# PKU-MARL/HARL

Hardware: AMD Instinct MI355X
Metric: transitions/sec through HAPPO update (MPE spread, 3 agents) (higher is better)
Workload: dtype f32; 1 GPU; MPE simple_spread_v2 3-agent HAPPO update: compute_returns + train(), T=200, n_rollout_threads=4096/GPU (4096 global, weak scaling), obs18/share54/Box5, MLP[128, 128], ppo_epoch=5, critic_epoch=5; episode_length=200, n_rollout_threads_per_gpu=4096, n_rollout_threads_global=4096, n_agents=3, parallelism=dp1, collective=none, world_size=1, ranks_seen=1

## Files before the change

harl_amd/csrc/heads_common.h:

```cpp
#pragma once
#include "common.h"

using namespace harl;

namespace {
constexpr float LOG_SQRT_2PI = 0.918938533204672741780329736406f;
constexpr float HALF_LOG_2PI_PLUS_HALF = 1.418938533204672741780329736406f;

struct ActorArgs {
  const float *xL;
  const uint32_t *relu_mask;
  const float *rstd;
  long M;
  const float *Whp, *bhp, *log_std;
  float std_x_coef, std_y_coef;
  int act_dim;
  const int64_t *idx;
  const float *actions, *avail, *old_logp, *adv;
  const double *adv_moments;
  const float *factor_in, *active;
  float clip_lo, clip_hi, entropy_coef;
  int agg_mean;
  float *dzL, *dhead, *part_scalars;
  float *dw_part;
// ... 75 lines not shown
        dx += dzh[4 * dq + 0] * w[0] + dzh[4 * dq + 1] * w[1] + dzh[4 * dq + 2] * w[2] + dzh[4 * dq + 3] * w[3];
      }
      const float da = rstd * (dx - s1 - xv[c] * s2);
      o[c] = (int)b0 < 0 ? da : 0.f;
      b0 <<= 1;
    }
    op[q * WAVE] = o;
    xv = xn;
  }
}

template <int H>
__device__ __forceinline__ void head_load_regs(const float *__restrict__ xL, long slab, int lane, f32x4 (&xs)[H / 8]) {
  const f32x4 *xp = reinterpret_cast<const f32x4 *>(xL + slab * (long)(H * SLAB)) + lane;
#pragma unroll
  for (int q = 0; q < H / 8; ++q) xs[q] = xp[q * WAVE];
}

template <int H, int DAP, int DA = DAP>
__device__ __forceinline__ void head_fwd_regs(const f32x4 (&xs)[H / 8], const float *whl_h, const float *cst,
                                              float (&z)[DAP]) {
#pragma unroll
  for (int d = 0; d < DAP; ++d) z[d] = 0.f;
#pragma unroll
  for (int q = 0; q < H / 8; ++q) {
#pragma unroll
    for (int c = 0; c < 4; ++c) {
#pragma unroll
      for (int dq = 0; dq < (DA + 3) / 4; ++dq) {
        const f32x4 w = *reinterpret_cast<const f32x4 *>(whl_h + (4 * q + c) * DAP + 4 * dq);
#pragma unroll
        for (int e = 0; e < 4; ++e)
          if (4 * dq + e < DA) z[4 * dq + e] += xs[q][c] * w[e];
      }
    }
    __builtin_amdgcn_sched_barrier(0);
  }
#pragma unroll
  for (int d = 0; d < DA; ++d) z[d] = wave_sum32(z[d]) + cst[d];
}

constexpr int HEAD_T_PAD = 16;
__host__ __device__ constexpr int head_t_rows(int da) { return 2 * ((da + 1) / 2); }
__host__ __device__ constexpr int head_t_block(int H, int da) { return head_t_rows(da) * (H / 2) + HEAD_T_PAD; }

template <int H, int DAP, int DA>
__device__ __forceinline__ void head_fwd_regs_t(const f32x4 (&xs)[H / 8], const float *whlT_h, const float *cst,
                                                float (&z)[DAP]) {
#pragma unroll
  for (int d = 0; d < DAP; ++d) z[d] = 0.f;
  f32x4 w[2][DA];
#pragma unroll
  for (int d = 0; d < DA; ++d) w[0][d] = *reinterpret_cast<const f32x4 *>(whlT_h + d * (H / 2));
#pragma unroll
  for (int q = 0; q < H / 8; ++q) {
    if (q + 1 < H / 8) {
#pragma unroll
      for (int d = 0; d < DA; ++d) w[(q + 1) & 1][d] = *reinterpret_cast<const f32x4 *>(whlT_h + d * (H / 2) + 4 * (q + 1));
    }
#pragma unroll
    for (int c = 0; c < 4; ++c)
#pragma unroll
      for (int d = 0; d < DA; ++d) z[d] += xs[q][c] * w[q & 1][d][c];
    __builtin_amdgcn_sched_barrier(0);
  }
#pragma unroll
  for (int d = 0; d < DA; ++d) z[d] = wave_sum32(z[d]) + cst[d];
}

template <int H, int DAP, int DA>
__device__ __forceinline__ void stage_head_t(float *whlT, float *cst, const float *__restrict__ Whp,
                                             const float *__restrict__ bhp, int n_threads) {
  constexpr int DAE = head_t_rows(DA), BLK = head_t_block(H, DA);
  for (int e = threadIdx.x; e < 2 * DAE * (H / 2); e += n_threads) {
    const int R = e % (H / 2), d = (e / (H / 2)) % DAE, hh = e / ((H / 2) * DAE);
    whlT[hh * BLK + d * (H / 2) + R] = d < DA ? Whp[d * H + feat_base(R) + 4 * hh] : 0.f;
  }
  for (int e = threadIdx.x; e < DAP; e += n_threads) {
    cst[e] = e < DA ? bhp[e] : 0.f;
    float rs = 0.f;
    if (e < DA)
      for (int f = 0; f < H; ++f) rs += Whp[e * H + f];
    cst[4 * DAP + e] = rs;
  }
}

template <int H, int DAP, int DA = DAP, bool PACKED = false, bool WT = false>
__device__ __forceinline__ void head_bwd_regs_bits(const f32x4 (&xs)[H / 8], uint32_t b0, const uint32_t b1, float rstd,
                                                   long slab, int lane, const float *whl ,
                                                   const float (&dzh)[DAP], float s1, float s2,
                                                   float *__restrict__ dz_out, const uint32_t bm1 = 0u,
                                                   const uint32_t bm2 = 0u) {
  s1 *= (1.0f / H);
  s2 *= (1.0f / H);
  const int i = lane & 31, h = lane >> 5;
  const float *wa = WT ? whl + ((i >> 2) & 1) * head_t_block(H, DA) + (i & 3) + 4 * (i >> 3) + h * (H / 2)
                       : whl + (((i >> 2) & 1) * (H / 2) + (i & 3) + 4 * (i >> 3)) * DAP + h;
  f32x16 acc[H / 32];
#pragma unroll
  for (int t = 0; t < H / 32; ++t)
#pragma unroll
    for (int r = 0; r < 16; ++r) acc[t][r] = 0.f;
#pragma unroll
  for (int st = 0; st < (DA + 1) / 2; ++st) {
    const unsigned hm = 0u - (unsigned)h;
    const float bsel = __uint_as_float((__float_as_uint(dzh[2 * st + 1]) & hm) | (__float_as_uint(dzh[2 * st]) & ~hm));
#pragma unroll
    for (int t = 0; t < H / 32; ++t)
      acc[t] = __builtin_amdgcn_mfma_f32_32x32x2f32(wa[WT ? 16 * t + 2 * st * (H / 2) : 16 * t * DAP + 2 * st], bsel, acc[t], 0, 0, 0);
  }
  f32x4 *op = reinterpret_cast<f32x4 *>(dz_out + slab * (long)(H * SLAB)) + lane;
  const float c1 = -s1 * rstd, c2 = -s2 * rstd;
  const f32x2 c1v = {c1, c1}, c2v = {c2, c2}, rv = {rstd, rstd};
#pragma unroll
  for (int q = 0; q < H / 8; ++q) {
    if (q == 8) b0 = H == 256 ? bm1 : b1;
    if (H == 256 && q == 16) b0 = bm2;
    if (H == 256 && q == 24) b0 = b1;
    f32x4 o;
    if constexpr (PACKED) {
#pragma unroll
      for (int P = 0; P < 2; ++P) {
        const int e = 4 * q + 2 * P;
        const f32x2 d = {acc[e >> 4][e & 15], acc[(e + 1) >> 4][(e + 1) & 15]}, x = {xs[q][2 * P], xs[q][2 * P + 1]};
        const f32x2 da = fma2(x, c2v, fma2(d, rv, c1v));
        o[2 * P] = mask_pop(da[0], b0);
        o[2 * P + 1] = mask_pop(da[1], b0);
      }
    } else {
#pragma unroll
      for (int c = 0; c < 4; ++c) {
        const float dx = acc[(4 * q + c) >> 4][(4 * q + c) & 15];
        const float da = rstd * (dx - s1 - xs[q][c] * s2);
        o[c] = (int)b0 < 0 ? da : 0.f;
        b0 <<= 1;
      }
    }
    op[q * WAVE] = o;
  }
}

template <int H, int DAP>
__device__ __forceinline__ void head_bwd_regs(const f32x4 (&xs)[H / 8], const uint32_t *__restrict__ mask_in,
                                              float rstd, long slab, int lane, const float *whl ,
                                              const float (&dzh)[DAP], float s1, float s2,
                                              float *__restrict__ dz_out) {
  constexpr int NW = (H / 2 + 31) / 32;
  const uint32_t b0 = mask_in[(slab * NW + 0) * WAVE + lane];
  const uint32_t b1 = NW > 1 ? mask_in[(slab * NW + (NW - 1)) * WAVE + lane] : 0u;
  const uint32_t bm1 = NW == 4 ? mask_in[(slab * NW + 1) * WAVE + lane] : 0u, bm2 = NW == 4 ? mask_in[(slab * NW + 2) * WAVE + lane] : 0u;
  head_bwd_regs_bits<H, DAP>(xs, b0, b1, rstd, slab, lane, whl, dzh, s1, s2, dz_out, bm1, bm2);
}

template <int H>
struct HeadDw {
  static constexpr int HX = 64 + 4;
  static constexpr int TD = 33;
  static constexpr int WAVE_FLOATS = SLAB * HX + SLAB * TD;
  static constexpr int OUT_FLOATS = 32 * H + 32;
};

template <int H, int DAP>
__device__ __forceinline__ void head_dw_step(const f32x4 (&xs)[H / 8], const float (&dzh)[DAP], float *tx, float *td,
                                             int lane, f32x16 (&acc)[H / 32]) {
  constexpr int HX = HeadDw<H>::HX, TD = HeadDw<H>::TD;
  const int i = lane & 31, h = lane >> 5;
  if (h == 0) {
#pragma unroll
    for (int d = 0; d < DAP; ++d) td[i * TD + d] = dzh[d];
  }
#pragma unroll
  for (int half = 0; half < H / 64; ++half) {
#pragma unroll
    for (int q = 0; q < 8; ++q)
      *reinterpret_cast<f32x4 *>(tx + i * HX + 32 * (q >> 2) + 8 * (q & 3) + 4 * h) = xs[8 * half + q];
    asm volatile("s_waitcnt lgkmcnt(0)" ::: "memory");
    __builtin_amdgcn_wave_barrier();
#pragma unroll
    for (int t = 0; t < SLAB / 2; ++t) {
      const float a = td[(2 * t + h) * TD + i];
#pragma unroll
      for (int n = 0; n < 2; ++n) {
        const float b = tx[(2 * t + h) * HX + 32 * n + i];
        acc[2 * half + n] = __builtin_amdgcn_mfma_f32_32x32x2f32(a, b, acc[2 * half + n], 0, 0, 0);
      }
    }
    asm volatile("s_waitcnt lgkmcnt(0)" ::: "memory");
    __builtin_amdgcn_wave_barrier();
  }
}

template <int H, int DAP, int HROWS>
__device__ __forceinline__ void head_dw_step_lds(const f32x4 (&xs)[H / 8], const float (&dzh)[DAP], float *tx, float *td,
                                                 int lane, float *hw) {
  constexpr int HX = HeadDw<H>::HX, TD = HeadDw<H>::TD;
  static_assert(HROWS <= 8, "rows 0..7 of a 16 x 16 tile live in the four registers of lane groups 0 and 1");
  const int i = lane & 31, h = lane >> 5;
  const int m16 = lane & 15, kg = lane >> 4;
  if (h == 0) {
#pragma unroll
    for (int d = 0; d < DAP; ++d) td[i * TD + d] = dzh[d];
  }
#pragma unroll
  for (int half = 0; half < H / 64; ++half) {
#pragma unroll
    for (int q = 0; q < 8; ++q)
      *reinterpret_cast<f32x4 *>(tx + i * HX + 32 * (q >> 2) + 8 * (q & 3) + 4 * h) = xs[8 * half + q];
    asm volatile("s_waitcnt lgkmcnt(0)" ::: "memory");
    __builtin_amdgcn_wave_barrier();
    f32x4 acc[4];
#pragma unroll
    for (int n = 0; n < 4; ++n) acc[n] = f32x4{0.f, 0.f, 0.f, 0.f};
#pragma unroll
    for (int t = 0; t < SLAB / 4; ++t) {
      const float a = td[(4 * t + kg) * TD + m16];
#pragma unroll
      for (int n = 0; n < 4; ++n) {
        const float b = tx[(4 * t + kg) * HX + 16 * n + m16];
        acc[n] = __builtin_amdgcn_mfma_f32_16x16x4f32(a, b, acc[n], 0, 0, 0);
      }
    }
#pragma unroll
    for (int n = 0; n < 4; ++n)
#pragma unroll
      for (int r = 0; r < 4; ++r) {
        if (r < HROWS && kg == 0) hw[r * H + 64 * half + 16 * n + m16] += acc[n][r];
        if (4 + r < HROWS && kg == 1) hw[(4 + r) * H + 64 * half + 16 * n + m16] += acc[n][r];
      }
    asm volatile("s_waitcnt lgkmcnt(0)" ::: "memory");
    __builtin_amdgcn_wave_barrier();
  }
}

template <int H, int DAP, int HROWS, int NWAVES>
__device__ __forceinline__ void head_dw_finish_lds(const float *hacc, float (&dbacc)[DAP], float *dbl,
                                                   float *__restrict__ out) {
  const int lane = threadIdx.x & 63, wave = wave_id();
  float dbs[DAP];
#pragma unroll
  for (int d = 0; d < DAP; ++d) dbs[d] = wave_reduce_sum(dbacc[d]);
  __syncthreads();
  if (lane == 0) {
#pragma unroll
    for (int d = 0; d < DAP; ++d) dbl[wave * PS_STRIDE + d] = dbs[d];
  }
  __syncthreads();
  for (int e = threadIdx.x; e < HeadDw<H>::OUT_FLOATS; e += 64 * NWAVES) {
    float t = 0.f;
    if (e < 32 * H) {
      const int row = e / H;
      if (row < HROWS) {
#pragma unroll
        for (int w = 0; w < NWAVES; ++w) t += hacc[(w * HROWS + row) * H + (e - row * H)];
      }
    } else {
      const int d = e - 32 * H;
      if (d < DAP) {
#pragma unroll
        for (int w = 0; w < NWAVES; ++w) t += dbl[w * PS_STRIDE + d];
      }
    }
    out[e] = t;
  }
}

template <int H, int DAP>
__device__ __forceinline__ void head_dw_finish(f32x16 (&acc)[H / 32], float (&dbacc)[DAP], float *buf ,
                                               float *__restrict__ out) {
  const int lane = threadIdx.x & 63, wave = wave_id();
  const int i = lane & 31, h = lane >> 5;
  float dbs[DAP];
#pragma unroll
  for (int d = 0; d < DAP; ++d) dbs[d] = wave_reduce_sum(dbacc[d]);
  __syncthreads();
  for (int w = 0; w < WAVES_PER_WG; ++w) {
    if (wave == w) {
#pragma unroll
      for (int n = 0; n < H / 32; ++n)
#pragma unroll
        for (int r = 0; r < 16; ++r) {
          const int o = (r & 3) + 8 * (r >> 2) + 4 * h;
          float *p = buf + o * H + 32 * n + i;
          *p = (w == 0 ? 0.f : *p) + acc[n][r];
        }
      if (lane < 32) {
        float v = 0.f;
#pragma unroll
        for (int d = 0; d < DAP; ++d)
          if (lane == d) v = dbs[d];
        float *p = buf + 32 * H + lane;
        *p = (w == 0 ? 0.f : *p) + v;
      }
    }
    __syncthreads();
  }
  for (int e = threadIdx.x; e < HeadDw<H>::OUT_FLOATS; e += WG_THREADS) out[e] = buf[e];
}

template <int DAP>
__device__ __forceinline__ void store_dhead(float *__restrict__ dhead, long slab, int lane, const float (&dzh)[DAP]) {
  const int i = lane & 31, h = lane >> 5;
  if constexpr (DAP <= 32) {
    float *dh = dhead + (slab * SLAB + i) * DHEAD_LD + 16 * h;
#pragma unroll
    for (int c = 0; c < 16; ++c) {
      float v0 = 0.f, v1 = 0.f;
// ... 359 lines not shown
```

harl_amd/csrc/update.hip:

```cpp
#include <type_traits>
#include "common.h"
#include "split_mfma.h"
#include "heads_common.h"
#include "mfma_transpose.h"
#include "../../include/harl_hip.h"

using namespace harl;

namespace {

int bad(const char *m) {
  set_error(m);
  return -2;
}

template <int H, bool MASK>
__device__ __forceinline__ void relu_ln(const f32x16 (&acc)[H / 32], float (&v)[H / 2], uint32_t (&bits)[(H / 2 + 31) / 32],
                                        float &rstd_out) {
  constexpr int NR = H / 2;
#pragma unroll
  for (int w = 0; w < (NR + 31) / 32; ++w) bits[w] = 0u;
#pragma unroll
  for (int R = 0; R < NR; ++R) {
    if constexpr (MASK) v[R] = relu_push(acc[R >> 4][R & 15], bits[R >> 5]);
// ... 89 lines not shown
  const long slab0 = (long)blockIdx.x * WAVES_PER_WG + wave, slab_stride = (long)gridDim.x * WAVES_PER_WG;
  const u32x4 *wl1 = w1img + lane;
  u32x4 *pk = park + (long)wave * (MT * 6 * 64) + lane;
  const Ident I = make_ident(lane);
  f32x16 acc2[MT][MT];
  float dbs[MT];
#pragma unroll
  for (int a = 0; a < MT; ++a) {
    dbs[a] = 0.f;
#pragma unroll
    for (int b = 0; b < MT; ++b)
#pragma unroll
      for (int r = 0; r < 16; ++r) acc2[a][b][r] = 0.f;
  }
  float xr[KP0 / 2];
  atl_load<KP0>(x0n, slab0 < n_slabs ? slab0 : 0, lane, xr);
  for (long slab = slab0; slab < n_slabs; slab += slab_stride) {
    float raw[NR];
    {
      u32x4 a1[NJ1], a2[NJ1], a3[NJ1];
      split_acts<KP0 / 2, false>(xr, a1, a2, a3);
      atl_load<H>(dz2, slab, lane, raw);
      atl_load<KP0>(x0n, slab + slab_stride < n_slabs ? slab + slab_stride : slab, lane, xr);
      float x1[NR];
      f32x16 acc[MT];
#pragma unroll
      for (int t = 0; t < MT; ++t)
#pragma unroll
        for (int r = 0; r < 16; ++r) acc[t][r] = b1l[32 * t + (r & 3) + 8 * (r >> 2) + 4 * h];
      split_gemm<MT, NJ1>(wl1, a1, a2, a3, acc, [](int) {});
      uint32_t bits[NW];
      float r1;
      relu_ln<H, false>(acc, x1, bits, r1);
#pragma unroll
      for (int b = 0; b < MT; ++b) {
        u32x4 B[3][2];
        split_transpose_block<false, false>(&x1[16 * b], I, B);
#pragma unroll
        for (int term = 0; term < 3; ++term)
#pragma unroll
          for (int ks = 0; ks < 2; ++ks) pk[((b * 3 + term) * 2 + ks) * 64] = B[term][ks];
      }
    }
    __builtin_amdgcn_sched_barrier(0);
    u32x4 A[MT][3][2];
#pragma unroll
    for (int a = 0; a < MT; ++a) dbs[a] += split_transpose_block<true, false>(&raw[16 * a], I, A[a]);
#pragma unroll
    for (int b = 0; b < MT; ++b) {
      u32x4 B[3][2];
#pragma unroll
      for (int term = 0; term < 3; ++term)
#pragma unroll
        for (int ks = 0; ks < 2; ++ks) B[term][ks] = pk[((b * 3 + term) * 2 + ks) * 64];
#pragma unroll
      for (int a = 0; a < MT; ++a) dw_tile(acc2[a][b], A[a], B);
    }
  }
  finish_partials<MT, MT>(acc2, dbs, reinterpret_cast<float *>(park), part, n_part_rows);
}

template <int H, int KP0>
__global__ __launch_bounds__(WG_THREADS, 1) void k_upd_dx(const float *__restrict__ x0n, const float *__restrict__ dz2,
                                                          const float *__restrict__ W1p, int D,
                                                          const float *__restrict__ b1p, const float *__restrict__ W2p,
                                                          long n_slabs, float *__restrict__ part, int n_part_rows) {
  extern __shared__ __attribute__((aligned(16))) float lds[];
  constexpr int MT = H / 32, KT = KP0 / 32, NJ1 = KP0 / 16, NJ2 = H / 16, NR = H / 2, NW = (NR + 31) / 32;
  u32x4 *img2 = reinterpret_cast<u32x4 *>(lds);
  u32x4 *w1img = img2 + 3 * MT * NJ2 * 64;
  float *b1l = reinterpret_cast<float *>(w1img + 3 * MT * NJ1 * 64);
  stage_split_matrix<H, H, true, WG_THREADS>(img2, W2p);
  stage_w1_images<H, KP0, WG_THREADS>(w1img, W1p, D);
  for (int e = threadIdx.x; e < H; e += WG_THREADS) b1l[e] = b1p[e];
  __syncthreads();
  const int lane = threadIdx.x & 63, wave = wave_id(), h = lane >> 5;
  const long slab0 = (long)blockIdx.x * WAVES_PER_WG + wave, slab_stride = (long)gridDim.x * WAVES_PER_WG;
  const u32x4 *wl1 = w1img + lane, *wl2 = img2 + lane;
  const Ident I = make_ident(lane);
  f32x16 acc1[MT][KT];
  float dbs[MT];
#pragma unroll
  for (int a = 0; a < MT; ++a) {
    dbs[a] = 0.f;
#pragma unroll
    for (int n = 0; n < KT; ++n)
#pragma unroll
      for (int r = 0; r < 16; ++r) acc1[a][n][r] = 0.f;
  }
  float raw[NR], xr[KP0 / 2];
  atl_load<H>(dz2, slab0 < n_slabs ? slab0 : 0, lane, raw);
  atl_load<KP0>(x0n, slab0 < n_slabs ? slab0 : 0, lane, xr);
  for (long slab = slab0; slab < n_slabs; slab += slab_stride) {
    u32x4 a1[NJ1], a2[NJ1], a3[NJ1];
    split_acts<KP0 / 2>(xr, a1, a2, a3);
    float dx[NR];
    {
      u32x4 g1[NJ2], g2[NJ2], g3[NJ2];
      split_acts<NR>(raw, g1, g2, g3);
      const long nxt = slab + slab_stride < n_slabs ? slab + slab_stride : slab;
      atl_load<H>(dz2, nxt, lane, raw);
      atl_load<KP0>(x0n, nxt, lane, xr);
      f32x16 acc[MT];
#pragma unroll
      for (int t = 0; t < MT; ++t)
#pragma unroll
        for (int r = 0; r < 16; ++r) acc[t][r] = 0.f;
      split_gemm<MT, NJ2>(wl2, g1, g2, g3, acc, [](int) {});
#pragma unroll
      for (int R = 0; R < NR; ++R) dx[R] = acc[R >> 4][R & 15];
    }
    float dz1[NR];
    {
      float x1[NR];
      uint32_t bits1[NW];
      float r1;
      f32x16 acc[MT];
#pragma unroll
      for (int t = 0; t < MT; ++t)
#pragma unroll
        for (int r = 0; r < 16; ++r) acc[t][r] = b1l[32 * t + (r & 3) + 8 * (r >> 2) + 4 * h];
      split_gemm<MT, NJ1>(wl1, a1, a2, a3, acc, [](int) {});
      relu_ln<H, true>(acc, x1, bits1, r1);
      ln_bwd_relu_bits<H>(dx, x1, bits1, r1, dz1);
    }
    u32x4 B[KT][3][2];
#pragma unroll
    for (int n = 0; n < KT; ++n)
      transpose_block<false>(a1[2 * n], a1[2 * n + 1], a2[2 * n], a2[2 * n + 1], a3[2 * n], a3[2 * n + 1], I, B[n]);
#pragma unroll
    for (int a = 0; a < MT; ++a) {
      u32x4 A[3][2];
      dbs[a] += split_transpose_block<true>(&dz1[16 * a], I, A);
#pragma unroll
      for (int n = 0; n < KT; ++n) dw_tile(acc1[a][n], A, B[n]);
    }
  }
  finish_partials<MT, KT>(acc1, dbs, reinterpret_cast<float *>(img2), part, n_part_rows);
}

struct UpdFwdArgs {
  const float *x0n, *W1p, *b1p, *W2p, *b2p;
  int D;
  long n_slabs;
  float *dz2;
  int n_part_rows;
  float *xh1;
  uint32_t *mask1;
  float *rstd1;
};

constexpr int UF_WAVES = 8, UF_THREADS = 64 * UF_WAVES;

template <int NV>
__device__ __forceinline__ void block_reduce_store8(float (&v)[NV], float *red , float *out_row) {
  const int lane = threadIdx.x & 63, wave = wave_id();
#pragma unroll
  for (int k = 0; k < NV; ++k) {
    float t = wave_reduce_sum(v[k]);
    if (lane == 0) red[wave * PS_STRIDE + k] = t;
  }
  __syncthreads();
  if (threadIdx.x < PS_STRIDE) {
    float t = 0.f;
    if (threadIdx.x < NV) {
#pragma unroll
      for (int w = 0; w < UF_WAVES; ++w) t += red[w * PS_STRIDE + threadIdx.x];
    }
    out_row[threadIdx.x] = t;
  }
}

template <int H, int KP0, int DA, bool DISCRETE, bool TRAIN, typename ARGS>
__global__ __launch_bounds__(UF_THREADS, 2) void k_upd_fwd(UpdFwdArgs U, ARGS A) {
  constexpr bool CRITIC = std::is_same<ARGS, CriticArgs>::value;
  static_assert(DA >= 1 && DA <= 8 && (!CRITIC || DA == 1), "the LDS head-gradient tile covers 8 head outputs");
  constexpr int DAP = DA <= 4 ? 4 : 8;
  constexpr int HROWS = DA;
  constexpr bool HID = KP0 == 0;
  constexpr bool EARLY_X0N = H == 128 && KP0 == 32 && DA <= 5 && !DISCRETE;
  constexpr bool EARLY_X0N_LP = !TRAIN && !HID && (H == 64 || (DA != 4 && !(KP0 == 64 && DA >= 7 && !DISCRETE)));
  static_assert(!HID || TRAIN, "the last-layer variant exists for optimiser steps only");
  extern __shared__ __attribute__((aligned(16))) float lds[];
  PHASE_BEGIN();
  constexpr int MT = H / 32, NJ1 = KP0 / 16, NJ2 = H / 16, NR = H / 2, NW = (NR + 31) / 32;
  u32x4 *w2img = reinterpret_cast<u32x4 *>(lds);
  u32x4 *w1img = w2img + 3 * MT * NJ2 * 64;
  float *b1l = reinterpret_cast<float *>(w1img + 3 * MT * NJ1 * 64);
  float *b2l = b1l + H;
  float *whlT = b2l + H;
  float *cst = whlT + 2 * head_t_block(H, DA);
  float *red = cst + 7 * DAP;
  float *hacc = red + UF_WAVES * PS_STRIDE;
  const int lane = threadIdx.x & 63, wave = wave_id(), i = lane & 31, h = lane >> 5;
  const long slab0 = (long)wave * gridDim.x + blockIdx.x, slab_stride = (long)gridDim.x * UF_WAVES;
  constexpr int NXR = HID ? NR : KP0 / 2;
  float xr[NXR];
  atl_load<2 * NXR>(U.x0n, slab0 < U.n_slabs ? slab0 : 0, lane, xr);
  constexpr bool ROWS = !CRITIC || TRAIN;
  long rawn = 0;
  if constexpr (ROWS) rawn = row_index_request(A.idx, A.Whp, slab0, lane, A.M);
  stage_split_matrix<H, H, false, UF_THREADS>(w2img, U.W2p);
  if constexpr (!HID) stage_w1_images<H, KP0, UF_THREADS>(w1img, U.W1p, U.D);
  for (int e = threadIdx.x; e < H; e += UF_THREADS) {
    if constexpr (!HID) b1l[e] = U.b1p[e];
    b2l[e] = U.b2p[e];
  }
  if (TRAIN)
    for (int e = threadIdx.x; e < UF_WAVES * HROWS * H; e += UF_THREADS) hacc[e] = 0.f;
  if (threadIdx.x < WG_THREADS) {
    stage_head_t<H, DAP, DA>(whlT, cst, A.Whp, A.bhp, WG_THREADS);
    if constexpr (!CRITIC) {
      if (!DISCRETE) {
        for (int e = threadIdx.x; e < DAP; e += WG_THREADS) {
          float sg = 0.5f, sig = 1.f, lsig = 0.f, dsd = 0.f;
          if (e < A.act_dim) {
            sg = 1.0f / (1.0f + expf(-A.log_std[e] / A.std_x_coef));
            sig = sg * A.std_y_coef;
            lsig = logf(sig);
            dsd = A.std_y_coef * sg * (1.f - sg) / A.std_x_coef;
          }
          cst[DAP + e] = sig;
          cst[2 * DAP + e] = lsig;
          cst[3 * DAP + e] = dsd;
          cst[5 * DAP + e] = 1.0f / sig;
          cst[6 * DAP + e] = 1.0f / (sig * sig);
        }
      }
    }
  }
  __syncthreads();

  const u32x4 *wl1 = w1img + lane, *wl2 = w2img + lane;
  const float *whlT_h = whlT + h * head_t_block(H, DA);
  float *hw = hacc + wave * (HROWS * H);

  float adv_mean = 0.f, adv_den = 1.f, vmean = 0.f, vsd = 1.f;
  if constexpr (CRITIC) {
    if (TRAIN && A.vn_stats) {
      const float d = fmaxf(A.vn_stats[2], 1e-5f);
      vmean = A.vn_stats[0] / d;
      const float msq = A.vn_stats[1] / d;
      vsd = sqrtf(fmaxf(msq - vmean * vmean, 1e-2f));
    }
  } else {
    if (TRAIN && A.adv_moments) {
      const double cnt = A.adv_moments[2];
      const double m = A.adv_moments[0] / cnt;
      const double var = A.adv_moments[1] / cnt - m * m;
      adv_mean = (float)m;
      adv_den = 1.0f / ((float)sqrt(var > 0 ? var : 0.0) + 1e-5f);
    }
  }
  adv_mean = uniform_f(adv_mean);
  adv_den = uniform_f(adv_den);
  vmean = uniform_f(vmean);
  vsd = uniform_f(vsd);
  constexpr int NSC = CRITIC ? 8 : 8 + DAP;
  float sc[NSC];
#pragma unroll
  for (int k = 0; k < NSC; ++k) sc[k] = 0.f;
  float dbacc[CRITIC ? DAP : 1];
#pragma unroll
  for (int d = 0; d < (CRITIC ? DAP : 1); ++d) dbacc[d] = 0.f;

  __builtin_amdgcn_s_waitcnt(0x0F70);
  PHASE(10);
  for (long slab = slab0; slab < U.n_slabs; slab += slab_stride) {
    ActorRow<DAP> rcur;
    float cvold = 0.f, cret = 0.f;
    if constexpr (ROWS) {
      const long row = row_index_resolve(A.idx, rawn, slab, lane, A.M);
      if constexpr (!CRITIC) actor_row_load_at<DAP, DISCRETE, TRAIN, DA>(A, slab, lane, row, rcur);
      else critic_row_load_at(A, row, cvold, cret);
      rawn = row_index_request(A.idx, A.Whp, slab + slab_stride, lane, A.M);
      __builtin_amdgcn_sched_barrier(0);
    }
    float v[NR];
    uint32_t bits2[NW];
    float r2;
    {
      float x1[NR];
      if constexpr (HID) {
#pragma unroll
        for (int R = 0; R < NR; ++R) x1[R] = xr[R];
        PHASE(0);
        PHASE(1);
      } else {
        u32x4 a1[NJ1], a2[NJ1], a3[NJ1];
        split_acts<KP0 / 2>(xr, a1, a2, a3);
        if constexpr (EARLY_X0N_LP) atl_load<2 * NXR>(U.x0n, slab + slab_stride < U.n_slabs ? slab + slab_stride : slab, lane, xr);
        f32x16 acc[MT];
#pragma unroll
        for (int t = 0; t < MT; ++t)
#pragma unroll
          for (int r = 0; r < 16; ++r) acc[t][r] = b1l[32 * t + (r & 3) + 8 * (r >> 2) + 4 * h];
        PHASE(0);
        split_gemm<MT, NJ1>(wl1, a1, a2, a3, acc, [](int) {});
        PHASE(1);
        uint32_t bits1[NW];
        float r1;
        relu_ln<H, TRAIN>(acc, x1, bits1, r1);
        if constexpr (TRAIN) {
          if (U.xh1) {
            atl_store<H>(U.xh1, slab, lane, x1);
#pragma unroll
            for (int w = 0; w < NW; ++w) U.mask1[(slab * NW + w) * WAVE + lane] = bits1[w];
            if (lane < 32) U.rstd1[slab * SLAB + lane] = r1;
          }
        }
      }
      u32x4 y1[NJ2], y2[NJ2], y3[NJ2];
      split_acts<NR>(x1, y1, y2, y3);
      PHASE(2);
      f32x16 acc[MT];
#pragma unroll
      for (int t = 0; t < MT; ++t)
#pragma unroll
        for (int r = 0; r < 16; ++r) acc[t][r] = b2l[32 * t + (r & 3) + 8 * (r >> 2) + 4 * h];
      split_gemm<MT, NJ2>(wl2, y1, y2, y3, acc, [](int) {});
      PHASE(3);
      relu_ln<H, TRAIN>(acc, v, bits2, r2);
    }
    PHASE(4);
    f32x4 xs[H / 8];
#pragma unroll
    for (int q = 0; q < H / 8; ++q) xs[q] = f32x4{v[4 * q], v[4 * q + 1], v[4 * q + 2], v[4 * q + 3]};
    float z[DAP];
    head_fwd_regs_t<H, DAP, DA>(xs, whlT_h, cst, z);
    PHASE(5);
    const long sn = slab + slab_stride < U.n_slabs ? slab + slab_stride : slab;
    if constexpr (!TRAIN && !EARLY_X0N_LP) atl_load<2 * NXR>(U.x0n, sn, lane, xr);
    float dzh[DAP];
    float s1, s2;
    if constexpr (CRITIC) {
      float dv;
      if (!critic_sample<TRAIN>(A, z[0], slab, lane, vmean, vsd, sc, dv, cvold, cret)) continue;
#pragma unroll
      for (int d = 0; d < DAP; ++d) dzh[d] = d == 0 ? dv : 0.f;
      s1 = dv * cst[4 * DAP];
      s2 = dv * (z[0] - cst[0]);
    } else {
      if (!actor_sample<DAP, DISCRETE, TRAIN, DA>(A, cst, z, slab, lane, adv_mean, adv_den, sc, dzh, s1, s2, rcur)) continue;
    }
    PHASE(6);
    if constexpr (TRAIN) {
      if constexpr (EARLY_X0N) atl_load<2 * NXR>(U.x0n, sn, lane, xr);
      int lane_o = lane;
      asm volatile("" : "+v"(lane_o));
      const Ident I = make_ident(lane_o);
      const u32x4 I16 = make_ident16(lane_o);
      u32x4 Ah[3][2];
      {
        float e8[8];
#pragma unroll
        for (int c = 0; c < 8; ++c) e8[c] = (c < DAP && h == 0) ? dzh[c < DAP ? c : 0] : 0.f;
        u32x4 t1, t2, t3;
#pragma unroll
        for (int c = 0; c < 4; ++c) {
          unsigned a, b, d;
          split3(e8[2 * c], e8[2 * c + 1], a, b, d);
          t1[c] = a;
          t2[c] = b;
          t3[c] = d;
        }
        const f32x16 zero = {0.f, 0.f, 0.f, 0.f, 0.f, 0.f, 0.f, 0.f, 0.f, 0.f, 0.f, 0.f, 0.f, 0.f, 0.f, 0.f};
        const f32x16 c1 = mfma_bf16(t1, I16, zero), c2 = mfma_bf16(t2, I16, zero), c3 = mfma_bf16(t3, I16, zero);
        pack_transposed(c1, Ah[0][0], Ah[0][1]);
        pack_transposed(c2, Ah[1][0], Ah[1][1]);
        pack_transposed(c3, Ah[2][0], Ah[2][1]);
      }
#pragma unroll
      for (int n = 0; n < MT; ++n) {
        u32x4 B[3][2];
        split_transpose_block<false>(&v[16 * n], I, B);
        f32x16 tile = {0.f, 0.f, 0.f, 0.f, 0.f, 0.f, 0.f, 0.f, 0.f, 0.f, 0.f, 0.f, 0.f, 0.f, 0.f, 0.f};
        dw_tile(tile, Ah, B);
#pragma unroll
        for (int r = 0; r < 4; ++r) {
          if (r < HROWS && h == 0) hw[r * H + 32 * n + i] += tile[r];
          if (4 + r < HROWS && h == 1) hw[(4 + r) * H + 32 * n + i] += tile[r];
        }
      }
      if constexpr (CRITIC) {
        if (h == 0) dbacc[0] += dzh[0];
      } else {
        if (h == 1) {
#pragma unroll
          for (int d = 0; d < DAP; ++d) sc[8 + d] += dzh[d];
        }
      }
      PHASE(7);
      if constexpr (!EARLY_X0N) atl_load<2 * NXR>(U.x0n, sn, lane, xr);
      head_bwd_regs_bits<H, DAP, DA, true, true>(xs, bits2[0], bits2[NW - 1], r2, slab, lane, whlT, dzh, s1, s2, U.dz2);
      PHASE(8);
    }
  }
  if constexpr (TRAIN) {
    float dbv[DAP];
#pragma unroll
    for (int d = 0; d < DAP; ++d) {
      if constexpr (CRITIC) {
        dbv[d] = dbacc[d];
      } else {
        dbv[d] = h == 1 ? sc[8 + d] : 0.f;
        sc[8 + d] = h == 0 ? sc[8 + d] : 0.f;
      }
    }
    block_reduce_store8<NSC>(sc, red, A.part_scalars + (long)blockIdx.x * PS_STRIDE);
    for (int row = blockIdx.x + gridDim.x; row < U.n_part_rows; row += gridDim.x)
      if (threadIdx.x < PS_STRIDE) A.part_scalars[(long)row * PS_STRIDE + threadIdx.x] = 0.f;
    float dbs[DAP];
#pragma unroll
    for (int d = 0; d < DAP; ++d) dbs[d] = wave_reduce_sum(dbv[d]);
    float *dbl = red;
    __syncthreads();
    if (lane == 0) {
#pragma unroll
      for (int d = 0; d < DAP; ++d) dbl[wave * PS_STRIDE + d] = dbs[d];
    }
    __syncthreads();
    float *out = A.dw_part + (long)blockIdx.x * HeadDw<H>::OUT_FLOATS;
    for (int e = threadIdx.x; e < HeadDw<H>::OUT_FLOATS; e += UF_THREADS) {
      float t = 0.f;
      if (e < 32 * H) {
        const int row = e / H;
        if (row < HROWS) {
#pragma unroll
          for (int w = 0; w < UF_WAVES; ++w) t += hacc[(w * HROWS + row) * H + (e - row * H)];
        }
      } else {
        const int d = e - 32 * H;
        if (d < DAP) {
#pragma unroll
          for (int w = 0; w < UF_WAVES; ++w) t += dbl[w * PS_STRIDE + d];
        }
      }
      out[e] = t;
    }
    for (int row = blockIdx.x + gridDim.x; row < U.n_part_rows; row += gridDim.x) {
      float *zr = A.dw_part + (long)row * HeadDw<H>::OUT_FLOATS;
      for (int e = threadIdx.x; e < HeadDw<H>::OUT_FLOATS; e += UF_THREADS) zr[e] = 0.f;
    }
  }
  PHASE(11);
  PHASE_END((TRAIN ? 0 : 2) + (CRITIC ? 1 : 0));
}

int fwd_grid(long n_slabs) {
  const long wgs = (n_slabs + UF_WAVES - 1) / UF_WAVES;
  return (int)(wgs < 256 ? (wgs < 1 ? 1 : wgs) : 256);
}

int upd_grid(long n_slabs) {
  const long wgs = (n_slabs + WAVES_PER_WG - 1) / WAVES_PER_WG;
  return (int)(wgs < 256 ? (wgs < 1 ? 1 : wgs) : 256);
}

size_t fwd_lds_bytes(int H, int kp0, int dap, int hrows, int da) {
  return split_image_bytes(H, H) + split_image_bytes(H, kp0) +
         ((size_t)2 * H + (size_t)2 * head_t_block(H, da) + 7 * dap + UF_WAVES * PS_STRIDE + (size_t)UF_WAVES * hrows * H) *
             sizeof(float);
}

constexpr size_t LDS_PER_WG_MAX = 160 * 1024;

template <int H, int KP0, int DA, bool DISC, bool TRAIN, typename ARGS>
int launch_fwd(const UpdFwdArgs &U, const ARGS &A, hipStream_t s) {
  const size_t shm = fwd_lds_bytes(H, KP0, DA <= 4 ? 4 : 8, TRAIN ? DA : 0, DA);
  if (shm > LDS_PER_WG_MAX) {
    return bad("harl_update_*: this (D, H, act_dim) does not fit the LDS of one workgroup");
  }
  allow_big_lds(k_upd_fwd<H, KP0, DA, DISC, TRAIN, ARGS>, shm);
  hipLaunchKernelGGL((k_upd_fwd<H, KP0, DA, DISC, TRAIN, ARGS>), dim3(fwd_grid(U.n_slabs)), dim3(UF_THREADS), shm, s, U, A);
  return 0;
}

template <int H, int KP0, bool TRAIN, int DA = 8>
int launch_actor_width(const UpdFwdArgs &U, const ActorArgs &A, int discrete, hipStream_t s) {
  if (A.act_dim == DA)
    return discrete ? launch_fwd<H, KP0, DA, true, TRAIN, ActorArgs>(U, A, s) : launch_fwd<H, KP0, DA, false, TRAIN, ActorArgs>(U, A, s);
  if constexpr (DA > 1) return launch_actor_width<H, KP0, TRAIN, DA - 1>(U, A, discrete, s);
  return bad("harl_update_*: act_dim must be in [1, 8]");
}

template <bool TRAIN>
int dispatch_fwd_actor(const UpdFwdArgs &U, const ActorArgs &A, int H, int discrete, hipStream_t s) {
  const int D = A.act_dim;
  if (D < 1 || D > 8) return bad("harl_update_fwd: act_dim must be in [1, 8]");
  const int kp0 = U.D <= 32 ? 32 : 64;
#define CASE(Hv, Kv)                                                                \
  if (H == Hv && kp0 == Kv) {                                                       \
    const int rc = launch_actor_width<Hv, Kv, TRAIN>(U, A, discrete, s);             \
    return rc ? rc : check_launch("harl_update_fwd");                               \
  }
  CASE(128, 32) CASE(128, 64) CASE(64, 32) CASE(64, 64)
#undef CASE
  return bad("harl_update_fwd: hidden width must be 64 or 128");
}

int dispatch_last_actor(const UpdFwdArgs &U, const ActorArgs &A, int H, int discrete, hipStream_t s) {
  const int D = A.act_dim;
  if (D < 1 || D > 8) return bad("harl_update_last_actor: act_dim must be in [1, 8]");
  int rc;
  if (H == 128) rc = launch_actor_width<128, 0, true>(U, A, discrete, s);
  else if (H == 64) rc = launch_actor_width<64, 0, true>(U, A, discrete, s);
  else return bad("harl_update_last_actor: hidden width must be 64 or 128");
  return rc ? rc : check_launch("harl_update_last_actor");
}

int dispatch_last_critic(const UpdFwdArgs &U, const CriticArgs &A, int H, hipStream_t s) {
  int rc;
  if (H == 128) rc = launch_fwd<128, 0, 1, false, true, CriticArgs>(U, A, s);
  else if (H == 64) rc = launch_fwd<64, 0, 1, false, true, CriticArgs>(U, A, s);
  else return bad("harl_update_last_critic: hidden width must be 64 or 128");
  return rc ? rc : check_launch("harl_update_last_critic");
}

template <bool TRAIN>
int dispatch_fwd_critic(const UpdFwdArgs &U, const CriticArgs &A, int H, hipStream_t s) {
  const int kp0 = U.D <= 32 ? 32 : 64;
#define CASE(Hv, Kv)                                                     \
  if (H == Hv && kp0 == Kv) {                                            \
    const int rc = launch_fwd<Hv, Kv, 1, false, TRAIN, CriticArgs>(U, A, s); \
    return rc ? rc : check_launch("harl_update_fwd");                        \
  }
  CASE(128, 32) CASE(128, 64) CASE(64, 32) CASE(64, 64)
#undef CASE
  return bad("harl_update_fwd: hidden width must be 64 or 128");
}

}

HARL_PHASE_ACCESSOR(update)

extern "C" int harl_update_supported(int D, int H, int act_dim, int kind) {
  if (!(D >= 0 && D <= 64 && (H == 64 || H == 128) && act_dim >= 1 && act_dim <= 8)) return 0;
  const int dap = act_dim <= 4 ? 4 : 8;
  const int hrows = kind == 0 ? 0 : (kind == 2 ? 1 : act_dim);
  return fwd_lds_bytes(H, D == 0 ? 0 : (D <= 32 ? 32 : 64), dap, hrows, kind == 2 ? 1 : act_dim) <= LDS_PER_WG_MAX ? 1 : 0;
}

extern "C" int harl_update_fwd_actor(const float *x0n, long M, int D, int H, const float *W1p, const float *b1p,
                                     const float *W2p, const float *b2p, const float *Whp, const float *bhp,
                                     const float *log_std, float std_x_coef, float std_y_coef, int discrete, int act_dim,
                                     const float *actions, const float *avail, const float *old_logp, const float *adv,
                                     const double *adv_moments, const float *factor, const float *active,
                                     double clip_param, float entropy_coef, int agg_mean, int trpo, float *logp_out,
                                     float *dz2, float *part_scalars, float *dw_part_head, int n_part_rows, float *xh1,
                                     uint32_t *rmask1, float *rstd1, void *stream) {
  if (M <= 0) return 0;
  if (D < 1 || D > 64) return bad("harl_update_fwd_actor: input width must be <= 64");
  if (!dz2 || !part_scalars || !dw_part_head || n_part_rows <= 0) return bad("harl_update_fwd_actor: missing outputs");
  if (xh1 && (!rmask1 || !rstd1)) return bad("harl_update_fwd_actor: xh1 needs rmask1 and rstd1");
  UpdFwdArgs U{x0n, W1p, b1p, W2p, b2p, D, n_slabs_of(M), dz2, n_part_rows, xh1, rmask1, rstd1};
  if (fwd_grid(U.n_slabs) > n_part_rows) return bad("harl_update_fwd_actor: n_part_rows smaller than the launch grid");
  ActorArgs A{};
  A.trpo = trpo;
  A.logp_out = logp_out;
  A.dw_part = dw_part_head;
  A.M = M; A.Whp = Whp; A.bhp = bhp; A.log_std = log_std;
  A.std_x_coef = std_x_coef; A.std_y_coef = std_y_coef; A.act_dim = act_dim;
  A.actions = actions; A.avail = avail; A.old_logp = old_logp; A.adv = adv; A.adv_moments = adv_moments;
  A.factor_in = factor; A.active = active; A.entropy_coef = entropy_coef;
  A.clip_lo = (float)(1.0 - clip_param); A.clip_hi = (float)(1.0 + clip_param);
  A.agg_mean = agg_mean; A.part_scalars = part_scalars; A.n_slabs = U.n_slabs;
  return dispatch_fwd_actor<true>(U, A, H, discrete, (hipStream_t)stream);
}

extern "C" int harl_update_logp(const float *x0n, long M, int D, int H, const float *W1p, const float *b1p,
                                const float *W2p, const float *b2p, const float *Whp, const float *bhp,
                                const float *log_std, float std_x_coef, float std_y_coef, int discrete, int act_dim,
                                const float *actions, const float *avail, float *logp_out, const float *old_logp,
                                float *factor, int agg_mean, float *head_out, void *stream) {
  if (M <= 0) return 0;
  if (D < 1 || D > 64) return bad("harl_update_logp: input width must be <= 64");
  if (factor && !old_logp) return bad("harl_update_logp: factor update needs old_logp");
  UpdFwdArgs U{x0n, W1p, b1p, W2p, b2p, D, n_slabs_of(M), nullptr, 0, nullptr, nullptr, nullptr};
  ActorArgs A{};
  A.head_out = head_out;
  A.M = M; A.Whp = Whp; A.bhp = bhp; A.log_std = log_std;
  A.std_x_coef = std_x_coef; A.std_y_coef = std_y_coef; A.act_dim = act_dim;
  A.actions = actions; A.avail = avail; A.old_logp = old_logp; A.agg_mean = agg_mean;
  A.logp_out = logp_out; A.factor_out = factor; A.n_slabs = U.n_slabs;
  return dispatch_fwd_actor<false>(U, A, H, discrete, (hipStream_t)stream);
}

extern "C" int harl_update_fwd_critic(const float *x0n, long M, int D, int H, const float *W1p, const float *b1p,
                                      const float *W2p, const float *b2p, const float *Whp, const float *bhp,
                                      const float *value_preds, const float *returns, const float *vn_stats,
                                      float clip_param, int use_clipped, int use_huber, float huber_delta, float *dz2,
                                      float *part_scalars, float *dw_part_head, int n_part_rows, float *xh1,
                                      uint32_t *rmask1, float *rstd1, void *stream) {
  if (M <= 0) return 0;
  if (D < 1 || D > 64) return bad("harl_update_fwd_critic: input width must be <= 64");
// ... 97 lines not shown
```

Before: 52.61 million transitions/s.

## Compute critic head weight gradient with DPP lane reduce-scatter instead of MFMA

For the critic training kernel, whose head has a single output, the head weight gradient is now formed as per-lane products dz*v. These are reduced across lanes with a DPP/permlane16 reduce-scatter, replacing the split-bf16 MFMA transpose path and its per-tile LDS accumulation. Each lane keeps a few accumulated sums in registers and writes them once at the end. The change also zeroes less LDS and turns on early x0n prefetch for this variant. The risks are extra VALU/DPP work per slab, higher register pressure, and a different summation order for the gradient.

```diff
diff --git a/harl_amd/csrc/heads_common.h b/harl_amd/csrc/heads_common.h
--- a/harl_amd/csrc/heads_common.h
+++ b/harl_amd/csrc/heads_common.h
@@ -251,6 +251,42 @@
   head_bwd_regs_bits<H, DAP>(xs, b0, b1, rstd, slab, lane, whl, dzh, s1, s2, dz_out, bm1, bm2);
 }
 
+constexpr int LANE_RS_BIT[5] = {3, 2, 1, 0, 4};
+template <int CTRL>
+__device__ __forceinline__ float dpp_partner(float x) {
+  return __uint_as_float((unsigned)__builtin_amdgcn_update_dpp(0, (int)__float_as_uint(x), CTRL, 0xf, 0xf, true));
+}
+template <int NOUT, int CTRL>
+__device__ __forceinline__ void lane_rs_step(const float *in, float *out, bool upper) {
+#pragma clang fp contract(off)
+#pragma unroll
+  for (int k = 0; k < NOUT; ++k) {
+    const float lo = in[k] + dpp_partner<CTRL>(in[k]), hi = in[k + NOUT] + dpp_partner<CTRL>(in[k + NOUT]);
+    out[k] = upper ? hi : lo;
+  }
+}
+template <int N>
+__device__ __forceinline__ int lane_rs_index(int lane, int k) {
+  int R = k;
+#pragma unroll
+  for (int s = 0; s < 5; ++s) R += ((lane >> LANE_RS_BIT[s]) & 1) * (N >> (s + 1));
+  return R;
+}
+template <int N>
+__device__ __forceinline__ void lane32_reduce_scatter(float (&p)[N], int lane, float (&out)[N / 32]) {
+  static_assert(N == 32 || N == 64, "one or two sums per lane");
+  float a[N / 2], b[N / 4], c[N / 8], d[N / 16];
+  lane_rs_step<N / 2, 0x128>(p, a, (lane & 8) != 0);
+  lane_rs_step<N / 4, 0x141>(a, b, (lane & 4) != 0);
+  lane_rs_step<N / 8, 0x4E>(b, c, (lane & 2) != 0);
+  lane_rs_step<N / 16, 0xB1>(c, d, (lane & 1) != 0);
+#pragma unroll
+  for (int k = 0; k < N / 32; ++k) {
+    const auto r = __builtin_amdgcn_permlane16_swap(__float_as_uint(d[k]), __float_as_uint(d[k + N / 32]), false, false);
+    out[k] = __uint_as_float(r[0]) + __uint_as_float(r[1]);
+  }
+}
+
 template <int H>
 struct HeadDw {
   static constexpr int HX = 64 + 4;
diff --git a/harl_amd/csrc/update.hip b/harl_amd/csrc/update.hip
--- a/harl_amd/csrc/update.hip
+++ b/harl_amd/csrc/update.hip
@@ -265,22 +265,29 @@
 
 constexpr int UF_WAVES = 8, UF_THREADS = 64 * UF_WAVES;
 
+#ifndef HARL_CRITIC_HEAD_DW_MFMA
+#define HARL_CRITIC_HEAD_DW_MFMA 0
+#endif
+#ifndef HARL_CRITIC_EARLY_X0N
+#define HARL_CRITIC_EARLY_X0N 1
+#endif
+
 template <int NV>
-__device__ __forceinline__ void block_reduce_store8(float (&v)[NV], float *red , float *out_row) {
-  const int lane = threadIdx.x & 63, wave = wave_id();
+__device__ __forceinline__ void block_reduce_store8(float (&v)[NV], float *red , float *out_row, int tid) {
+  const int lane = tid & 63, wave = wave_id();
 #pragma unroll
   for (int k = 0; k < NV; ++k) {
     float t = wave_reduce_sum(v[k]);
     if (lane == 0) red[wave * PS_STRIDE + k] = t;
   }
   __syncthreads();
-  if (threadIdx.x < PS_STRIDE) {
+  if (tid < PS_STRIDE) {
     float t = 0.f;
-    if (threadIdx.x < NV) {
-#pragma unroll
-      for (int w = 0; w < UF_WAVES; ++w) t += red[w * PS_STRIDE + threadIdx.x];
-    }
-    out_row[threadIdx.x] = t;
+    if (tid < NV) {
+#pragma unroll
+      for (int w = 0; w < UF_WAVES; ++w) t += red[w * PS_STRIDE + tid];
+    }
+    out_row[tid] = t;
   }
 }
 
@@ -290,8 +297,9 @@
   static_assert(DA >= 1 && DA <= 8 && (!CRITIC || DA == 1), "the LDS head-gradient tile covers 8 head outputs");
   constexpr int DAP = DA <= 4 ? 4 : 8;
   constexpr int HROWS = DA;
+  constexpr bool LANE_DW = CRITIC && TRAIN && !HARL_CRITIC_HEAD_DW_MFMA;
   constexpr bool HID = KP0 == 0;
-  constexpr bool EARLY_X0N = H == 128 && KP0 == 32 && DA <= 5 && !DISCRETE;
+  constexpr bool EARLY_X0N = (H == 128 && KP0 == 32 && DA <= 5 && !DISCRETE) || (LANE_DW && HARL_CRITIC_EARLY_X0N);
   constexpr bool EARLY_X0N_LP = !TRAIN && !HID && (H == 64 || (DA != 4 && !(KP0 == 64 && DA >= 7 && !DISCRETE)));
   static_assert(!HID || TRAIN, "the last-layer variant exists for optimiser steps only");
   extern __shared__ __attribute__((aligned(16))) float lds[];
@@ -319,7 +327,7 @@
     if constexpr (!HID) b1l[e] = U.b1p[e];
     b2l[e] = U.b2p[e];
   }
-  if (TRAIN)
+  if (TRAIN && !LANE_DW)
     for (int e = threadIdx.x; e < UF_WAVES * HROWS * H; e += UF_THREADS) hacc[e] = 0.f;
   if (threadIdx.x < WG_THREADS) {
     stage_head_t<H, DAP, DA>(whlT, cst, A.Whp, A.bhp, WG_THREADS);
@@ -376,6 +384,9 @@
   float dbacc[CRITIC ? DAP : 1];
 #pragma unroll
   for (int d = 0; d < (CRITIC ? DAP : 1); ++d) dbacc[d] = 0.f;
+  float hdw[LANE_DW ? NR / 32 : 1];
+#pragma unroll
+  for (int k = 0; k < (LANE_DW ? NR / 32 : 1); ++k) hdw[k] = 0.f;
 
   __builtin_amdgcn_s_waitcnt(0x0F70);
   PHASE(10);
@@ -459,40 +470,50 @@
     PHASE(6);
     if constexpr (TRAIN) {
       if constexpr (EARLY_X0N) atl_load<2 * NXR>(U.x0n, sn, lane, xr);
-      int lane_o = lane;
-      asm volatile("" : "+v"(lane_o));
-      const Ident I = make_ident(lane_o);
-      const u32x4 I16 = make_ident16(lane_o);
-      u32x4 Ah[3][2];
-      {
-        float e8[8];
-#pragma unroll
-        for (int c = 0; c < 8; ++c) e8[c] = (c < DAP && h == 0) ? dzh[c < DAP ? c : 0] : 0.f;
-        u32x4 t1, t2, t3;
-#pragma unroll
-        for (int c = 0; c < 4; ++c) {
-          unsigned a, b, d;
-          split3(e8[2 * c], e8[2 * c + 1], a, b, d);
-          t1[c] = a;
-          t2[c] = b;
-          t3[c] = d;
+      if constexpr (LANE_DW) {
+        float pr[NR];
+#pragma unroll
+        for (int R = 0; R < NR; ++R) pr[R] = dzh[0] * v[R];
+        float sl[NR / 32];
+        lane32_reduce_scatter<NR>(pr, lane, sl);
+#pragma unroll
+        for (int k = 0; k < NR / 32; ++k) hdw[k] += sl[k];
+      } else {
+        int lane_o = lane;
+        asm volatile("" : "+v"(lane_o));
+        const Ident I = make_ident(lane_o);
+        const u32x4 I16 = make_ident16(lane_o);
+        u32x4 Ah[3][2];
+        {
+          float e8[8];
+#pragma unroll
+          for (int c = 0; c < 8; ++c) e8[c] = (c < DAP && h == 0) ? dzh[c < DAP ? c : 0] : 0.f;
+          u32x4 t1, t2, t3;
+#pragma unroll
+          for (int c = 0; c < 4; ++c) {
+            unsigned a, b, d;
+            split3(e8[2 * c], e8[2 * c + 1], a, b, d);
+            t1[c] = a;
+            t2[c] = b;
+            t3[c] = d;
+          }
+          const f32x16 zero = {0.f, 0.f, 0.f, 0.f, 0.f, 0.f, 0.f, 0.f, 0.f, 0.f, 0.f, 0.f, 0.f, 0.f, 0.f, 0.f};
+          const f32x16 c1 = mfma_bf16(t1, I16, zero), c2 = mfma_bf16(t2, I16, zero), c3 = mfma_bf16(t3, I16, zero);
+          pack_transposed(c1, Ah[0][0], Ah[0][1]);
+          pack_transposed(c2, Ah[1][0], Ah[1][1]);
+          pack_transposed(c3, Ah[2][0], Ah[2][1]);
         }
-        const f32x16 zero = {0.f, 0.f, 0.f, 0.f, 0.f, 0.f, 0.f, 0.f, 0.f, 0.f, 0.f, 0.f, 0.f, 0.f, 0.f, 0.f};
-        const f32x16 c1 = mfma_bf16(t1, I16, zero), c2 = mfma_bf16(t2, I16, zero), c3 = mfma_bf16(t3, I16, zero);
-        pack_transposed(c1, Ah[0][0], Ah[0][1]);
-        pack_transposed(c2, Ah[1][0], Ah[1][1]);
-        pack_transposed(c3, Ah[2][0], Ah[2][1]);
-      }
-#pragma unroll
-      for (int n = 0; n < MT; ++n) {
-        u32x4 B[3][2];
-        split_transpose_block<false>(&v[16 * n], I, B);
-        f32x16 tile = {0.f, 0.f, 0.f, 0.f, 0.f, 0.f, 0.f, 0.f, 0.f, 0.f, 0.f, 0.f, 0.f, 0.f, 0.f, 0.f};
-        dw_tile(tile, Ah, B);
-#pragma unroll
-        for (int r = 0; r < 4; ++r) {
-          if (r < HROWS && h == 0) hw[r * H + 32 * n + i] += tile[r];
-          if (4 + r < HROWS && h == 1) hw[(4 + r) * H + 32 * n + i] += tile[r];
+#pragma unroll
+        for (int n = 0; n < MT; ++n) {
+          u32x4 B[3][2];
+          split_transpose_block<false>(&v[16 * n], I, B);
+          f32x16 tile = {0.f, 0.f, 0.f, 0.f, 0.f, 0.f, 0.f, 0.f, 0.f, 0.f, 0.f, 0.f, 0.f, 0.f, 0.f, 0.f};
+          dw_tile(tile, Ah, B);
+#pragma unroll
+          for (int r = 0; r < 4; ++r) {
+            if (r < HROWS && h == 0) hw[r * H + 32 * n + i] += tile[r];
+            if (4 + r < HROWS && h == 1) hw[(4 + r) * H + 32 * n + i] += tile[r];
+          }
         }
       }
       if constexpr (CRITIC) {
@@ -510,31 +531,37 @@
     }
   }
   if constexpr (TRAIN) {
+    const int lane_e = (int)__builtin_amdgcn_mbcnt_hi(~0u, __builtin_amdgcn_mbcnt_lo(~0u, 0u)), h_e = lane_e >> 5;
+    const int tid = wave * WAVE + lane_e;
+    if constexpr (LANE_DW) {
+#pragma unroll
+      for (int k = 0; k < NR / 32; ++k) hw[feat_base(lane_rs_index<NR>(lane_e, k)) + 4 * h_e] = hdw[k];
+    }
     float dbv[DAP];
 #pragma unroll
     for (int d = 0; d < DAP; ++d) {
       if constexpr (CRITIC) {
         dbv[d] = dbacc[d];
       } else {
-        dbv[d] = h == 1 ? sc[8 + d] : 0.f;
-        sc[8 + d] = h == 0 ? sc[8 + d] : 0.f;
+        dbv[d] = h_e == 1 ? sc[8 + d] : 0.f;
+        sc[8 + d] = h_e == 0 ? sc[8 + d] : 0.f;
       }
     }
-    block_reduce_store8<NSC>(sc, red, A.part_scalars + (long)blockIdx.x * PS_STRIDE);
+    block_reduce_store8<NSC>(sc, red, A.part_scalars + (long)blockIdx.x * PS_STRIDE, tid);
     for (int row = blockIdx.x + gridDim.x; row < U.n_part_rows; row += gridDim.x)
-      if (threadIdx.x < PS_STRIDE) A.part_scalars[(long)row * PS_STRIDE + threadIdx.x] = 0.f;
+      if (tid < PS_STRIDE) A.part_scalars[(long)row * PS_STRIDE + tid] = 0.f;
     float dbs[DAP];
 #pragma unroll
     for (int d = 0; d < DAP; ++d) dbs[d] = wave_reduce_sum(dbv[d]);
     float *dbl = red;
     __syncthreads();
-    if (lane == 0) {
+    if (lane_e == 0) {
 #pragma unroll
       for (int d = 0; d < DAP; ++d) dbl[wave * PS_STRIDE + d] = dbs[d];
     }
     __syncthreads();
     float *out = A.dw_part + (long)blockIdx.x * HeadDw<H>::OUT_FLOATS;
-    for (int e = threadIdx.x; e < HeadDw<H>::OUT_FLOATS; e += UF_THREADS) {
+    for (int e = tid; e < HeadDw<H>::OUT_FLOATS; e += UF_THREADS) {
       float t = 0.f;
       if (e < 32 * H) {
         const int row = e / H;
@@ -553,7 +580,7 @@
     }
     for (int row = blockIdx.x + gridDim.x; row < U.n_part_rows; row += gridDim.x) {
       float *zr = A.dw_part + (long)row * HeadDw<H>::OUT_FLOATS;
-      for (int e = threadIdx.x; e < HeadDw<H>::OUT_FLOATS; e += UF_THREADS) zr[e] = 0.f;
+      for (int e = tid; e < HeadDw<H>::OUT_FLOATS; e += UF_THREADS) zr[e] = 0.f;
     }
   }
   PHASE(11);
```

After: 53.12 million transitions/s (median of 6 runs). About the same (+1.0%).
